# liuzuxin/FSRL

Measured on NVIDIA H100. Metric: env-steps/sec (collect+update) SafetyCarCircle-v0 PPO-Lag, higher is better.
Workload: dtype f32

## Files before the change

### fsrl_b200/csrc/ppo_persist.cu

```cuda
#include "ppo_persist.cuh"
#include "arena.cuh"
#include "ppo_loss.cuh"
#include "wgmma.cuh"
#include <cstdlib>
#include <cmath>
#include <vector>

namespace fsrl {
namespace pp {

using namespace wg;

constexpr int WQ = 2;
constexpr int NEPI = 128 * WQ;
constexpr int TPB = NEPI + 32;
constexpr int C1 = 16 / WQ;
constexpr int C2 = 32 / WQ;
constexpr int RB = 64;
constexpr int MB = 256;
constexpr int KC = 32, NCH = 256 / KC;
constexpr int SLOT_BYTES = 32768, NSLOT = 4;
constexpr int A_CHUNK = 64 * KC * 4;
constexpr int ACC_LD = 68;
constexpr int OUTP = 8;
constexpr int H_ = 256;
constexpr int IMG = 65536;
enum { I_H1A_HI, I_H1A_LO, I_H1T_HI, I_H1T_LO, I_DZA_HI, I_DZA_LO, I_DZT_HI, I_DZT_LO, I_W2A_HI, I_W2A_LO, I_W2B_HI, I_W2B_LO, N_IMG };
constexpr int DB2P_OFF = N_IMG * IMG;
constexpr int DW3P_OFF = DB2P_OFF + 4 * H_;
constexpr int DB3P_OFF = DW3P_OFF + 4 * H_ * OUTP;
constexpr int MAXD = 40;
constexpr int NSMAX = (MAXD + 1) * 32 + 32 + 32 * OUTP + 16;
constexpr int SLICE_OFF = DB3P_OFF + 4 * 16;
constexpr int NET_WS = SLICE_OFF + 8 * NSMAX;
constexpr int SUMSQ_FLOATS = 128;
constexpr int FLAG_LINE = 32;
constexpr int F_A = 0, F_C = 1, F_PER_NET = 2;
constexpr int TILE_PK = (64 * 64 / NEPI + 2) / 3;
constexpr int TILE_FLOATS = TILE_PK * NEPI * 4;
constexpr int SLICE_PK = (NSMAX + 2) / 3;
constexpr int XG_PER_NET = 16 * TILE_FLOATS + 8 * SLICE_PK * 4;
constexpr int MAX_MB = 16384;
constexpr long long WAIT_CYCLES = 6000000000LL;

struct Args {
    fsrl_ppo_update_t u;
    int n_mb, slot0;
    long long adam_t0;
    float* ws;
    unsigned* flags;
    int* err;
    const float* adam_tab;
    long long* dbg;
    int dbg_step;
    unsigned dp_seq;
    int dp_direct;
};
constexpr int DBG_N = 48;
#define STAMP(i) do { if (P.dbg && t == P.dbg_step) P.dbg[(size_t)blockIdx.x * DBG_N + (i)] = clock64(); } while (0)

struct AdamS { float w1, b2, w2, rbc2s, eps, neg_step; };
__device__ __forceinline__ float adam_one(float p, float g, float& m, float& v, const AdamS& a) {
    m = m + a.w1 * (g - m);
    v = v * a.b2 + (a.w2 * g) * g;
    const float sq = v > 0.f ? v * rsqrtf(v) : 0.f;
    const float denom = fmaf(sq, a.rbc2s, a.eps);
    return p + __fdividef(a.neg_step * m, denom);
}

__device__ __forceinline__ void fail(int* err, int code) {
    *reinterpret_cast<volatile int*>(err) = code;
    __threadfence_system();
    asm volatile("trap;");
}
__device__ __forceinline__ uint32_t pk_hash(float x, float y, float z) {
    const uint32_t a = __float_as_uint(x), b = __float_as_uint(y), c = __float_as_uint(z);
    return a ^ __funnelshift_l(b, b, 11) ^ __funnelshift_l(c, c, 22);
}
__device__ __forceinline__ bool pk_ok(const float4& v, uint32_t tag) { return (__float_as_uint(v.w) ^ pk_hash(v.x, v.y, v.z)) == tag; }
__device__ __forceinline__ void st_packet(float* p, float x, float y, float z, uint32_t tag) {
    asm volatile("st.relaxed.sys.global.v4.f32 [%0], {%1,%2,%3,%4};" ::"l"(p), "f"(x), "f"(y), "f"(z), "f"(__uint_as_float(tag ^ pk_hash(x, y, z))) : "memory");
}
__device__ __forceinline__ float4 ld_packet(const float* p) {
    float4 v;
    asm volatile("ld.relaxed.sys.global.v4.f32 {%0,%1,%2,%3}, [%4];" : "=f"(v.x), "=f"(v.y), "=f"(v.z), "=f"(v.w) : "l"(p) : "memory");
    return v;
}

__device__ __noinline__ float3 dp_gather(const float* src, long long stride, int me, int world, uint32_t tag,
                                        float ox, float oy, float oz, int* err, int code) {
    const long long t0w = clock64();
    float ax = 0.f, ay = 0.f, az = 0.f;
    for (int r0 = 0; r0 < world; r0 += 4) {
        float4 v[4];
        bool ok;
        do {
            ok = true;
#pragma unroll
            for (int k = 0; k < 4; ++k)
                if (r0 + k < world && r0 + k != me) v[k] = ld_packet(src + (size_t)(r0 + k) * stride);
#pragma unroll
            for (int k = 0; k < 4; ++k)
                if (r0 + k < world && r0 + k != me) ok = ok && pk_ok(v[k], tag);
            if (!ok && clock64() - t0w > 4 * WAIT_CYCLES) fail(err, code);
        } while (!ok);
#pragma unroll
        for (int k = 0; k < 4; ++k) {
            if (r0 + k >= world) continue;
            if (r0 + k == me) { ax += ox; ay += oy; az += oz; }
            else { ax += v[k].x; ay += v[k].y; az += v[k].z; }
        }
    }
    return make_float3(ax, ay, az);
}
__device__ __noinline__ void dp_push_all(const float* const* xg, size_t off, int me, int world, float x, float y, float z, uint32_t tag) {
    for (int r = 0; r < world; ++r)
        if (r != me) st_packet(const_cast<float*>(xg[r]) + off, x, y, z, tag);
}

__device__ __forceinline__ uint32_t mapa_u32(uint32_t local_saddr, uint32_t rank) {
// ... 218 lines not shown
__device__ __noinline__ float dp_tile_finish(DpCtx d, size_t off, float* accs, int trow, int cb2, int et) {
    float g[C2];
    const long long t0w = clock64();
    if (d.direct) {
        float own[C2];
        acc_ld<C2>(accs, trow, cb2, own);
#pragma unroll
        for (int jq = 0; jq < C2; ++jq) g[jq] = 0.f;
        for (int r = 0; r < d.world; ++r) {
            if (r == d.me) {
#pragma unroll
                for (int jq = 0; jq < C2; ++jq) g[jq] += own[jq];
                continue;
            }
            const float* src = d.xg[d.me] + (size_t)r * d.region + off;
            float4 v[TILE_PK];
            bool ok;
            do {
                ok = true;
#pragma unroll
                for (int q = 0; q < TILE_PK; ++q) v[q] = ld_packet(src + (size_t)q * NEPI * 4);
#pragma unroll
                for (int q = 0; q < TILE_PK; ++q) ok = ok && pk_ok(v[q], d.tag);
                if (!ok && clock64() - t0w > 4 * WAIT_CYCLES) fail(d.err, 42);
            } while (!ok);
#pragma unroll
            for (int q = 0; q < TILE_PK; ++q) {
                g[3 * q] += v[q].x;
                if (3 * q + 1 < C2) g[3 * q + 1] += v[q].y;
                if (3 * q + 2 < C2) g[3 * q + 2] += v[q].z;
            }
        }
        const float inv_world = 1.0f / (float)d.world;
        float sq = 0.f;
#pragma unroll
        for (int jq = 0; jq < C2; ++jq) { g[jq] *= inv_world; sq = fmaf(g[jq], g[jq], sq); }
        acc_st<C2>(accs, trow, cb2, g);
        return sq;
    }
    const float* res = d.xg[d.me] + (size_t)FSRL_P2P_MAX_RANKS * d.region + off;
    acc_ld<C2>(accs, trow, cb2, g);
    float4 v[TILE_PK];
    bool ok;
    do {
        ok = true;
#pragma unroll
        for (int q = 0; q < TILE_PK; ++q)
            if (dp_owner(et, q, d.world) != d.me) v[q] = ld_packet(res + (size_t)q * NEPI * 4);
#pragma unroll
        for (int q = 0; q < TILE_PK; ++q)
            if (dp_owner(et, q, d.world) != d.me) ok = ok && pk_ok(v[q], d.tag);
        if (!ok && clock64() - t0w > 4 * WAIT_CYCLES) fail(d.err, 42);
    } while (!ok);
    float sq = 0.f;
#pragma unroll
    for (int q = 0; q < TILE_PK; ++q) {
        if (dp_owner(et, q, d.world) == d.me) continue;
        g[3 * q] = v[q].x;
        if (3 * q + 1 < C2) g[3 * q + 1] = v[q].y;
        if (3 * q + 2 < C2) g[3 * q + 2] = v[q].z;
    }
#pragma unroll
    for (int jq = 0; jq < C2; ++jq) sq = fmaf(g[jq], g[jq], sq);
    acc_st<C2>(accs, trow, cb2, g);
    return sq;
}
__device__ __noinline__ void dp_slices(DpCtx d, size_t off_s, float* sp_g, int n, int et) {
    const int n3 = (n + 2) / 3;
    const float inv_world = 1.0f / (float)d.world;
    for (int i = et; i < n3; i += NEPI)
        dp_push_all(d.xg, (size_t)d.me * d.region + off_s + 4 * (size_t)i, d.me, d.world,
                    sp_g[3 * i], 3 * i + 1 < n ? sp_g[3 * i + 1] : 0.f, 3 * i + 2 < n ? sp_g[3 * i + 2] : 0.f, d.tag);
    const float* loc = d.xg[d.me];
    for (int i = et; i < n3; i += NEPI) {
        const float3 s3 = dp_gather(loc + off_s + 4 * (size_t)i, d.region, d.me, d.world, d.tag, sp_g[3 * i],
                                    3 * i + 1 < n ? sp_g[3 * i + 1] : 0.f, 3 * i + 2 < n ? sp_g[3 * i + 2] : 0.f, d.err, 40);
        sp_g[3 * i] = s3.x * inv_world;
        if (3 * i + 1 < n) sp_g[3 * i + 1] = s3.y * inv_world;
        if (3 * i + 2 < n) sp_g[3 * i + 2] = s3.z * inv_world;
    }
}

__device__ __forceinline__ bool red_cta() { return ((blockIdx.x >> 3) & 3) == ((blockIdx.x & 7) >> 2); }

__device__ __noinline__ float dp_tail(DpCtx d, size_t off_t, size_t off_s, float* accs, float* sp_g, int n, int trow, int cb2,
                                      int et, bool tile, bool slice) {
    if (tile && !d.direct) dp_tile_reduce(d, off_t, accs, trow, cb2, et);
    if (slice) dp_slices(d, off_s, sp_g, n, et);
    __syncwarp();
    return tile ? dp_tile_finish(d, off_t, accs, trow, cb2, et) : 0.f;
}

template <bool DP>
__global__ void __launch_bounds__(TPB, 1) ppo_persist_kernel(const Args P) {
    extern __shared__ __align__(1024) unsigned char smem_raw[];
    __shared__ __align__(8) uint64_t bar_full[NSLOT], bar_empty[NSLOT], bar_b, bar_w1;
    __shared__ float s_red[4][320];
    __shared__ float s_misc[32];
    __shared__ AdamS s_adam;
    __shared__ const float* s_xg[2][FSRL_P2P_MAX_RANKS];
    const fsrl_ppo_update_t& u = P.u;
    const int tid = threadIdx.x, warp = tid >> 5, lane = tid & 31;
    const int net = blockIdx.x >> 5, c = blockIdx.x & 31, a = c >> 3, b = c & 7;
    const bool is_g2 = c < 16;
    const int ka = (c & 15) >> 2, q4 = c & 3;

    const int D = u.D, A = u.A, C = u.C, H = H_;
    const int out = (net == 0) ? A : 1;
    const int n_cta = 32 * u.n_nets;
    float* wsn = P.ws + (size_t)net * NET_WS;
    float* sumsq_g = P.ws + (size_t)u.n_nets * NET_WS;
    unsigned* fl_net = P.flags + (size_t)net * F_PER_NET * FLAG_LINE;
    unsigned* fl_d2 = P.flags + (size_t)u.n_nets * F_PER_NET * FLAG_LINE;
    unsigned char* ring = smem_raw;
    float* accs = reinterpret_cast<float*>(smem_raw + NSLOT * SLOT_BYTES);
    float* small = accs + 64 * ACC_LD;
    const SliceMap sm(D);
    float* sp_p = small;
    float* sp_m = small + sm.n;
    float* sp_v = small + 2 * sm.n;
    float* sp_g = small + 3 * sm.n;
    float* land = small + 4 * sm.n;

    if (tid == 0) {
        for (int i = 0; i < NSLOT; ++i) { mbar_init(&bar_full[i], 1); mbar_init(&bar_empty[i], 4 * 8); }
        mbar_init(&bar_b, 1);
        mbar_init(&bar_w1, 4);
        fence_mbar_init();
    }
    __syncthreads();
    if (DP && threadIdx.x < 2 * FSRL_P2P_MAX_RANKS) s_xg[threadIdx.x / FSRL_P2P_MAX_RANKS][threadIdx.x % FSRL_P2P_MAX_RANKS] = P.u.p2p_xg[threadIdx.x / FSRL_P2P_MAX_RANKS][threadIdx.x % FSRL_P2P_MAX_RANKS];
    if (DP) __syncthreads();
    cluster_sync_all();

    const long long pbase = u.net_off[net];
    const ArenaLayout L = arena_layout(D, H, out, 0);
    const long long o_w1 = pbase + L.w1, o_b1 = pbase + L.b1, o_w2 = pbase + L.w2, o_b2 = pbase + L.b2,
                    o_w3 = pbase + L.w3, o_b3 = pbase + L.b3, o_ls = pbase + L.extra;

    if (warp == NEPI / 32) {
        if (elect_one()) {
            unsigned qq = 0;
            for (int t = 0; t < P.n_mb; ++t) {
                if (!flag_wait_ge<true>(fl_net + F_A * FLAG_LINE, 32u * (t + 1), WAIT_CYCLES)) fail(P.err, 10);
                STAMP(12);
                fence_proxy_async();
#pragma unroll 1
                for (int j = 0; j < NCH; ++j, ++qq) {
                    const int s = qq % NSLOT;
                    if (!mbar_wait(&bar_empty[s], ((qq / NSLOT) & 1) ^ 1, WAIT_CYCLES)) fail(P.err, 11);
                    unsigned char* dst = ring + (size_t)s * SLOT_BYTES;
                    mbar_expect_tx(&bar_full[s], 3 * A_CHUNK);
                    const size_t ao = (size_t)a * 16384 + (size_t)j * 64 * KC, bo = (size_t)b * 8192 + (size_t)j * 32 * KC;
                    copy_operand(dst, wsn + (size_t)I_H1A_HI * IMG + ao, A_CHUNK, &bar_full[s], 8, b, 0xff);
                    copy_operand(dst + 2 * A_CHUNK, wsn + (size_t)I_W2A_HI * IMG + bo, A_CHUNK / 2, &bar_full[s], 1, 0, 0);
                }
                STAMP(13);
                if (!flag_wait_ge<true>(fl_net + F_C * FLAG_LINE, 32u * (t + 1), WAIT_CYCLES)) fail(P.err, 12);
                STAMP(14);
                fence_proxy_async();
                const int ia = is_g2 ? I_W2B_HI : I_DZT_HI, ib = is_g2 ? I_DZA_HI : I_H1T_HI;
                const int blk_a = is_g2 ? ka : q4, blk_b = is_g2 ? q4 : ka;
                const uint16_t m4 = (uint16_t)(0xfu << (b & 4)), m2 = (uint16_t)(0x11u << (b & 3));
#pragma unroll 1
                for (int j = 0; j < NCH; ++j, ++qq) {
                    const int s = qq % NSLOT;
                    if (!mbar_wait(&bar_empty[s], ((qq / NSLOT) & 1) ^ 1, WAIT_CYCLES)) fail(P.err, 13);
                    unsigned char* dst = ring + (size_t)s * SLOT_BYTES;
                    mbar_expect_tx(&bar_full[s], 4 * A_CHUNK);
                    const size_t ao = (size_t)blk_a * 16384 + (size_t)j * 64 * KC, bo = (size_t)blk_b * 16384 + (size_t)j * 64 * KC;
                    copy_operand(dst, wsn + (size_t)ia * IMG + ao, A_CHUNK, &bar_full[s], is_g2 ? 4 : 2, is_g2 ? b & 3 : b >> 2, is_g2 ? m4 : m2);
                    copy_operand(dst + 2 * A_CHUNK, wsn + (size_t)ib * IMG + bo, A_CHUNK, &bar_full[s], is_g2 ? 2 : 4, is_g2 ? b >> 2 : b & 3, is_g2 ? m2 : m4);
                }
            }
        }
    } else {
        const int et = tid;
        const int sp = warp & 3;
        const int wq = warp >> 2;
        const int r16 = lane & 15, half = lane >> 4;
        const int trow = 16 * sp + r16;
        const int cb1 = 16 * half + C1 * wq;
        const int cb2 = 32 * half + C2 * wq;
        unsigned qq = 0;
        const uint32_t empty_r = mapa_u32(smem_u32(bar_empty), lane < 8 ? lane : 0);
        float w2p[C2], w2m[C2], w2v[C2];
        const int world = DP ? u.world : 1;
        auto dp_ctx = [&](int t_) {
            DpCtx d;
            const unsigned long long id = (unsigned long long)(P.adam_t0 + t_ + 1);
            d.xg = s_xg[(int)(id & 1ULL)];
            d.region = (long long)u.n_nets * XG_PER_NET;
            d.me = u.p2p_rank; d.world = world;
            d.tag = (P.dp_seq << 16) | (uint32_t)((t_ + 1) & 0xffff);
            d.err = P.err;
            d.direct = P.dp_direct;
            return d;
        };

        for (int i = et; i < sm.n; i += NEPI) {
            long long src = -1;
            if (i < sm.b2) { const int d = i / 32, kk = i % 32; src = (d < D) ? o_w1 + (long long)d * H + 32 * b + kk : o_b1 + 32 * b + kk; }
            else if (i < sm.w3) src = o_b2 + 32 * b + (i - sm.b2);
            else if (i < sm.b3) { const int oo = (i - sm.w3) / OUTP, jj = (i - sm.w3) % OUTP; if (jj < out) src = o_w3 + (long long)(32 * b + oo) * out + jj; }
            else { const int jj = i - sm.b3; if (jj < out) src = o_b3 + jj; else if (net == 0 && jj >= 8 && jj < 8 + A) src = o_ls + (jj - 8); }
            sp_p[i] = src >= 0 ? u.theta[src] : 0.f;
            sp_m[i] = src >= 0 ? u.adam_m[src] : 0.f;
            sp_v[i] = src >= 0 ? u.adam_v[src] : 0.f;
            sp_g[i] = 0.f;
        }
        if (!is_g2) {
            const int o = 64 * q4 + trow;
#pragma unroll
            for (int j = 0; j < C2; ++j) {
                const long long idx = o_w2 + (long long)(64 * ka + cb2 + j) * H + o;
                w2p[j] = u.theta[idx]; w2m[j] = u.adam_m[idx]; w2v[j] = u.adam_v[idx];
            }
        } else {
#pragma unroll
            for (int j = 0; j < C2; ++j) w2p[j] = w2m[j] = w2v[j] = 0.f;
        }
        epi_bar();

        for (int t = 0; t < P.n_mb; ++t) {
            const long long row0 = (long long)t * MB;
            const int slot = P.slot0 + t;
            if (et == 0) {
                s_adam.w1 = (float)(1.0 - u.beta1); s_adam.b2 = (float)u.beta2; s_adam.w2 = (float)(1.0 - u.beta2);
                s_adam.rbc2s = __ldg(P.adam_tab + 2 * t); s_adam.eps = (float)u.adam_eps; s_adam.neg_step = __ldg(P.adam_tab + 2 * t + 1);
                STAMP(0);
                if (P.dbg && t == P.dbg_step) { long long gt; asm volatile("mov.u64 %0, %%globaltimer;" : "=l"(gt)); P.dbg[(size_t)blockIdx.x * DBG_N + 30] = gt; }
                if (P.dbg && t == P.dbg_step + 64) {
                    long long gt; asm volatile("mov.u64 %0, %%globaltimer;" : "=l"(gt));
                    P.dbg[(size_t)blockIdx.x * DBG_N + 31] = gt;
                    P.dbg[(size_t)blockIdx.x * DBG_N + 29] = clock64();
                }
            }
            if (t + 1 < P.n_mb && et < 64) {
                const long long r = row0 + MB + 64 * a + et;
                prefetch_l2(u.obs + r * D);
                if (D > 32) prefetch_l2(u.obs + r * D + 32);
                if (is_g2) { prefetch_l2(u.obs + (r + 128) * D); if (D > 32) prefetch_l2(u.obs + (r + 128) * D + 32); }
                if (net == 0) { prefetch_l2(u.act + r * A); prefetch_l2(u.logp_old + r); prefetch_l2(u.adv + r); if (C > 1) prefetch_l2(u.adv + u.ld + r); }
                else { prefetch_l2(u.ret + (long long)(net - 1) * u.ld + r); if (u.value_clip) prefetch_l2(u.values + (long long)(net - 1) * u.ld + r); }
            }
            float* scratch = reinterpret_cast<float*>(ring);
            if (!is_g2) {
                const float (&pv)[C2] = w2p;
                float phi[C2], plo[C2];
                const int o = 64 * q4 + trow;
                float* w2a_hi = wsn + (size_t)I_W2A_HI * IMG + (size_t)(o >> 5) * 8192 + (size_t)(o & 31) * 4;
                float* w2a_lo = w2a_hi + IMG;
#pragma unroll
                for (int q = 0; q < C2 / 4; ++q) {
                    float4 hi, lo;
                    tf32_split(pv[4 * q], hi.x, lo.x); tf32_split(pv[4 * q + 1], hi.y, lo.y);
                    tf32_split(pv[4 * q + 2], hi.z, lo.z); tf32_split(pv[4 * q + 3], hi.w, lo.w);
                    const size_t plane = (size_t)(16 * ka + (cb2 >> 2) + q) * 128;
                    *reinterpret_cast<float4*>(w2a_hi + plane) = hi;
                    *reinterpret_cast<float4*>(w2a_lo + plane) = lo;
                    phi[4 * q] = hi.x; phi[4 * q + 1] = hi.y; phi[4 * q + 2] = hi.z; phi[4 * q + 3] = hi.w;
                    plo[4 * q] = lo.x; plo[4 * q + 1] = lo.y; plo[4 * q + 2] = lo.z; plo[4 * q + 3] = lo.w;
                }
                store_transposed<C2, 64>(scratch, phi, plo, trow, cb2, et, wsn + (size_t)I_W2B_HI * IMG + (size_t)ka * 16384, 64 * q4, 0);
            }
            if (is_g2) {
                const int r = et & 63, kc = C1 * (et >> 6);
                const float* x0 = u.obs + (row0 + 64 * a + r) * D;
                const float* x1 = u.obs + (row0 + 64 * (a + 2) + r) * D;
                float acc2[2][C1];
#pragma unroll
                for (int j = 0; j < C1; ++j) acc2[0][j] = acc2[1][j] = sp_p[sm.w1 + D * 32 + kc + j];
                for (int d = 0; d < D; ++d) {
                    const float xv0 = __ldg(x0 + d), xv1 = __ldg(x1 + d);
                    const float* w = sp_p + sm.w1 + d * 32 + kc;
#pragma unroll
                    for (int j = 0; j < C1; ++j) { acc2[0][j] = fmaf(xv0, w[j], acc2[0][j]); acc2[1][j] = fmaf(xv1, w[j], acc2[1][j]); }
                }
                constexpr int TSCR = 2 * 32 * 65;
#pragma unroll
                for (int rep = 0; rep < 2; ++rep) {
                    const int aa = a + 2 * rep;
                    float hi[C1], lo[C1];
                    float* a_hi = wsn + (size_t)I_H1A_HI * IMG + (size_t)aa * 16384 + (size_t)r * 4;
#pragma unroll
                    for (int q = 0; q < C1 / 4; ++q) {
#pragma unroll
                        for (int e = 0; e < 4; ++e) tf32_split(fmaxf(acc2[rep][4 * q + e], 0.f), hi[4 * q + e], lo[4 * q + e]);
                        const size_t plane = (size_t)(8 * b + (kc >> 2) + q) * 256;
                        *reinterpret_cast<float4*>(a_hi + plane) = make_float4(hi[4 * q], hi[4 * q + 1], hi[4 * q + 2], hi[4 * q + 3]);
                        *reinterpret_cast<float4*>(a_hi + IMG + plane) = make_float4(lo[4 * q], lo[4 * q + 1], lo[4 * q + 2], lo[4 * q + 3]);
                    }
                    transposed_stage<C1, 32>(scratch + rep * TSCR, hi, lo, r, kc);
                }
                epi_bar();
#pragma unroll
                for (int rep = 0; rep < 2; ++rep)
                    transposed_flush<32>(scratch + rep * TSCR, et, wsn + (size_t)I_H1T_HI * IMG + (size_t)(b >> 1) * 16384, 64 * (a + 2 * rep), 32 * (b & 1));
            }
            fence_proxy_async_smem();
            epi_bar();
            if (et == 0) { STAMP(1); flag_add_release(fl_net + F_A * FLAG_LINE); }

            const long long grow = row0 + 64 * a + trow;
            float p_act[8], p_lpo = 0.f, p_adv0 = 0.f, p_adv1 = 0.f, p_ret = 0.f, p_val = 0.f, mean[2] = {0.f, 0.f}, rstd[2] = {1.f, 1.f};
#pragma unroll
            for (int j = 0; j < 8; ++j) p_act[j] = 0.f;
            if (net == 0) {
#pragma unroll
                for (int j = 0; j < 8; ++j) if (j < A) p_act[j] = __ldg(u.act + grow * A + j);
                p_lpo = __ldg(u.logp_old + grow);
                p_adv0 = __ldg(u.adv + grow);
                if (C > 1) p_adv1 = __ldg(u.adv + u.ld + grow);
                const float* ms = u.mb_stats + (size_t)t * 4;
                mean[0] = __ldg(ms); rstd[0] = __ldg(ms + 1); mean[1] = __ldg(ms + 2); rstd[1] = __ldg(ms + 3);
            } else {
                p_ret = __ldg(u.ret + (long long)(net - 1) * u.ld + grow);
                if (u.value_clip) p_val = __ldg(u.values + (long long)(net - 1) * u.ld + grow);
            }
            float p_ls[8], p_rsg[8];
#pragma unroll
            for (int j = 0; j < 8; ++j) {
                p_ls[j] = (net == 0 && j < A) ? sp_p[sm.b3 + 8 + j] : 0.f;
                p_rsg[j] = 1.0f / expf(p_ls[j]);
            }

            {
                float dm[16], dc[16];
                if (wq == 0) gemm_phase<32>(ring, qq, bar_full, empty_r, dm, dc, P.err, 30, lane);
                else qq += NCH;
                stage_acc<32>(accs, dm, dc, wq, sp, lane);
            }
            if (et == 0) STAMP(2);
            float h2[C1];
            acc_ld<C1>(accs, trow, cb1, h2);
            float hp[OUTP];
#pragma unroll
            for (int j = 0; j < OUTP; ++j) hp[j] = 0.f;
#pragma unroll
            for (int j = 0; j < C1; ++j) {
                h2[j] = fmaxf(h2[j] + sp_p[sm.b2 + cb1 + j], 0.f);
                const float* w = sp_p + sm.w3 + (cb1 + j) * OUTP;
#pragma unroll
                for (int jj = 0; jj < OUTP; ++jj) hp[jj] = fmaf(h2[j], w[jj], hp[jj]);
            }
#pragma unroll
            for (int jj = 0; jj < OUTP; ++jj) hp[jj] += __shfl_xor_sync(0xffffffffu, hp[jj], 16);
            if (WQ > 1) {
                float* xh = &s_red[0][0];
                if (half == 0 && wq > 0) {
#pragma unroll
                    for (int jj = 0; jj < OUTP; ++jj) xh[((wq - 1) * 64 + trow) * OUTP + jj] = hp[jj];
                }
                epi_bar();
                if (half == 0 && wq == 0) {
#pragma unroll
                    for (int w2 = 1; w2 < WQ; ++w2)
#pragma unroll
                        for (int jj = 0; jj < OUTP; ++jj) hp[jj] += xh[((w2 - 1) * 64 + trow) * OUTP + jj];
                }
            }
            float outv[OUTP];
#pragma unroll
            for (int jj = 0; jj < OUTP; ++jj) outv[jj] = sp_p[sm.b3 + jj];
            if (et == 0) {
                STAMP(3);
                mbar_expect_tx(&bar_b, 8u * 64u * OUTP * (uint32_t)sizeof(float));
            }
            if (half == 0 && wq == 0) {
                const uint32_t mine = smem_u32(land + ((size_t)b * 64 + trow) * OUTP);
                const uint32_t bb_ = smem_u32(&bar_b);
#pragma unroll
                for (int r = 0; r < 8; ++r) {
                    const uint32_t ra = mapa_u32(mine, r), rb = mapa_u32(bb_, r);
                    st_async4(ra, make_float4(hp[0], hp[1], hp[2], hp[3]), rb);
                    st_async4(ra + 16, make_float4(hp[4], hp[5], hp[6], hp[7]), rb);
                }
            }
            if (!mbar_wait_cluster(&bar_b, t & 1, WAIT_CYCLES)) fail(P.err, 31);
            __syncwarp();
            if (et == 0) STAMP(4);
#pragma unroll
            for (int bb = 0; bb < 8; ++bb) {
                const float* src = land + ((size_t)bb * 64 + trow) * OUTP;
                const float4 v0 = *reinterpret_cast<const float4*>(src);
                const float4 v1 = *reinterpret_cast<const float4*>(src + 4);
                outv[0] += v0.x; outv[1] += v0.y; outv[2] += v0.z; outv[3] += v0.w;
                outv[4] += v1.x; outv[5] += v1.y; outv[6] += v1.z; outv[7] += v1.w;
            }
            float dd[16];
#pragma unroll
            for (int j = 0; j < 16; ++j) dd[j] = 0.f;
            float st_a = 0.f, st_b = 0.f, st_c = 0.f, st_d = 0.f;
            {
                const float invB = 1.0f / (float)MB;
                if (net == 0) {
                    float g_mu[8], g_ls[8];
                    ppo_actor_row(u, outv, p_act, p_ls, p_rsg, p_lpo, p_adv0, p_adv1, mean, rstd, invB, g_mu, g_ls,
                                  st_a, st_b, st_c);
#pragma unroll
                    for (int j = 0; j < 8; ++j) { dd[j] = g_mu[j]; dd[8 + j] = g_ls[j]; }
                } else {
                    dd[0] = ppo_value_row(u, outv[0], p_ret, p_val, invB, st_d);
                }
            }
            if (et == 0) STAMP(26);
            const int nfeed = (net == 0) ? A : 1;
            float dz[C1];
#pragma unroll
            for (int j = 0; j < C1; ++j) {
                const float* w = sp_p + sm.w3 + (cb1 + j) * OUTP;
                float g = 0.f;
#pragma unroll
                for (int jj = 0; jj < OUTP; ++jj) if (jj < nfeed) g = fmaf(dd[jj], w[jj], g);
                dz[j] = h2[j] > 0.f ? g : 0.f;
            }
            {
                float hi[C1], lo[C1];
                float* a_hi = wsn + (size_t)I_DZA_HI * IMG + (size_t)a * 16384 + (size_t)trow * 4;
#pragma unroll
                for (int q = 0; q < C1 / 4; ++q) {
#pragma unroll
                    for (int e = 0; e < 4; ++e) tf32_split(dz[4 * q + e], hi[4 * q + e], lo[4 * q + e]);
                    const size_t plane = (size_t)(8 * b + (cb1 >> 2) + q) * 256;
                    *reinterpret_cast<float4*>(a_hi + plane) = make_float4(hi[4 * q], hi[4 * q + 1], hi[4 * q + 2], hi[4 * q + 3]);
                    *reinterpret_cast<float4*>(a_hi + IMG + plane) = make_float4(lo[4 * q], lo[4 * q + 1], lo[4 * q + 2], lo[4 * q + 3]);
                }
                store_transposed<C1, 32>(scratch, hi, lo, trow, cb1, et, wsn + (size_t)I_DZT_HI * IMG + (size_t)(b >> 1) * 16384, 64 * a, 32 * (b & 1));
            }
            if (et == 0) STAMP(27);
            {
                float* row = &s_red[sp][0];
#pragma unroll
                for (int j = 0; j < C1; ++j) {
                    const float sdz = half_sum(dz[j]);
                    if (r16 == 0) row[cb1 + j] = sdz;
                }
#pragma unroll
                for (int jj = 0; jj < OUTP; ++jj) {
                    if (jj < nfeed) {
#pragma unroll
                        for (int j = 0; j < C1; ++j) {
                            const float sv = half_sum(h2[j] * dd[jj]);
                            if (r16 == 0) row[32 + 32 * jj + cb1 + j] = sv;
                        }
                    }
                }
                if (b == 0 && wq == 0) {
#pragma unroll
                    for (int j = 0; j < 16; ++j) {
                        const float sv = half_sum(dd[j]);
                        if (lane == 0) row[288 + j] = sv;
                    }
                    const float sa = half_sum(st_a), sb = half_sum(st_b), sc = half_sum(st_c), sdv = half_sum(st_d);
                    if (lane == 0) { row[304] = sa; row[305] = sb; row[306] = sc; row[307] = sdv; }
                }
            }
            epi_bar();
            if (et == 0) STAMP(28);
            for (int i = et; i < 32 + 32 * nfeed; i += NEPI) {
                const float tot = ((s_red[0][i] + s_red[1][i]) + s_red[2][i]) + s_red[3][i];
                if (i < 32) wsn[DB2P_OFF + a * H + 32 * b + i] = tot;
                else wsn[DW3P_OFF + ((size_t)a * H + 32 * b + ((i - 32) & 31)) * OUTP + ((i - 32) >> 5)] = tot;
            }
            if (b == 0) {
                if (et < 20) {
                    const int i = 288 + et;
                    const float tot = ((s_red[0][i] + s_red[1][i]) + s_red[2][i]) + s_red[3][i];
                    if (et < 16) wsn[DB3P_OFF + a * 16 + et] = tot;
                    else {
                        float* stat = u.stats + (size_t)slot * FSRL_PPO_STATS;
                        if (net == 0) { if (et == 16) atomicAdd(stat + ST_ACTOR_REW, tot); if (et == 17) atomicAdd(stat + ST_ACTOR_SAFETY, tot); if (et == 18) atomicAdd(stat + ST_KL, tot); }
                        else if (et == 19) atomicAdd(stat + ST_VF0 + (net - 1), tot);
                    }
                }
                if (net == 0 && a == 0 && et == 20) u.stats[(size_t)slot * FSRL_PPO_STATS + ST_ENTROPY] = ppo_entropy(sp_p + sm.b3 + 8, A);
            }
            fence_proxy_async_smem();
            epi_bar();
            if (et == 0) { STAMP(5); flag_add_release(fl_net + F_C * FLAG_LINE); }

            unsigned mbits = 0;
            if (is_g2) {
                const int k = 64 * ka + trow;
                const float* msk = wsn + (size_t)I_H1A_HI * IMG + (size_t)q4 * 16384 + (size_t)(k >> 2) * 256 + (k & 3);
                float mreg[C2];
#pragma unroll
                for (int jq = 0; jq < C2; ++jq) mreg[jq] = __ldcg(msk + (size_t)(cb2 + jq) * 4);
                float xr[(64 * MAXD + NEPI - 1) / NEPI];
                const int nx = (64 * D + NEPI - 1) / NEPI;
                const float* xb = u.obs + (row0 + 64 * q4) * D;
#pragma unroll
                for (int q = 0; q < (64 * MAXD + NEPI - 1) / NEPI; ++q)
                    xr[q] = (q < nx && et + q * NEPI < 64 * D) ? __ldg(xb + et + q * NEPI) : 0.f;
#pragma unroll
                for (int jq = 0; jq < C2; ++jq) mbits |= (mreg[jq] > 0.f ? 1u : 0u) << jq;
#pragma unroll
                for (int q = 0; q < (64 * MAXD + NEPI - 1) / NEPI; ++q) {
                    const int e = et + q * NEPI;
                    if (q < nx && e < 64 * D) { const int r = e / D; land[e + (r >> 5)] = xr[q]; }
                }
            }
            if (red_cta() && wq == 1) {
                const int tw = et - 128;
                if (tw == 0) {
                    if (!flag_wait_ge(fl_net + F_C * FLAG_LINE, 32u * (t + 1), WAIT_CYCLES)) fail(P.err, 35);
                    STAMP(15);
                }
                asm volatile("bar.sync 6, 128;" ::: "memory");
                for (int i0 = sm.b2 + tw; i0 < sm.n; i0 += 4 * 128) {
                    float pv[4][4];
#pragma unroll
                    for (int e = 0; e < 4; ++e) {
                        const int i = i0 + e * 128;
                        const float* src = wsn;
                        size_t stride = 0;
                        bool real = false;
                        if (i < sm.n) {
                            if (i < sm.w3) { src = wsn + DB2P_OFF + 32 * b + (i - sm.b2); stride = H; real = true; }
                            else if (i < sm.b3) {
                                const int oo = (i - sm.w3) / OUTP, jj = (i - sm.w3) % OUTP;
                                real = jj < out;
                                src = wsn + DW3P_OFF + ((size_t)32 * b + oo) * OUTP + jj; stride = (size_t)H * OUTP;
                            } else {
                                const int jj = i - sm.b3;
                                real = (jj < out) || (net == 0 && jj >= 8 && jj < 8 + A);
                                src = wsn + DB3P_OFF + jj; stride = 16;
                            }
                        }
#pragma unroll
                        for (int q = 0; q < 4; ++q) pv[e][q] = real ? __ldcg(src + q * stride) : 0.f;
                    }
#pragma unroll
                    for (int e = 0; e < 4; ++e) {
                        const int i = i0 + e * 128;
                        if (i < sm.n) {
                            float gsum = 0.f;
#pragma unroll
                            for (int q = 0; q < 4; ++q) gsum += pv[e][q];
                            sp_g[i] = gsum;
                        }
                    }
                }
                if (tw == 0) STAMP(16);
            }
            {
                float dm[32], dc[32];
                if (wq == 0) gemm_phase<64>(ring, qq, bar_full, empty_r, dm, dc, P.err, 32, lane);
                else qq += NCH;
                stage_acc<64>(accs, dm, dc, wq, sp, lane);
            }
            if (et == 0) STAMP(6);
            float sq = 0.f;
            if (is_g2) {
                float v[C2];
                acc_ld<C2>(accs, trow, cb2, v);
#pragma unroll
                for (int jq = 0; jq < C2; ++jq) v[jq] = ((mbits >> jq) & 1u) ? v[jq] : 0.f;
                epi_bar();
                if (et == 0) STAMP(22);
                const float* xh = land + (size_t)cb2 * D + half;
                float* dst = reinterpret_cast<float*>(ring) + (size_t)wq * (D + 1) * 64 + trow;
                for (int d = 0; d < D; ++d) {
                    float sacc = 0.f;
#pragma unroll
                    for (int jq = 0; jq < C2; ++jq) sacc = fmaf(xh[jq * D + d], v[jq], sacc);
                    sacc += __shfl_xor_sync(0xffffffffu, sacc, 16);
                    if (half == 0) dst[d * 64] = sacc;
                }
                float sb1 = 0.f;
#pragma unroll
                for (int jq = 0; jq < C2; ++jq) sb1 += v[jq];
                sb1 += __shfl_xor_sync(0xffffffffu, sb1, 16);
                if (half == 0) dst[D * 64] = sb1;
                if (et == 0) STAMP(23);
                epi_bar();
                if (et == 0) {
                    mbar_arrive_release_cluster(mapa_u32(smem_u32(&bar_w1), 2 * ka));
                    mbar_arrive_release_cluster(mapa_u32(smem_u32(&bar_w1), 2 * ka + 1));
                }
            } else {
                float g[C2];
                acc_ld<C2>(accs, trow, cb2, g);
                if (DP) {
                    dp_tile_send(dp_ctx(t), (size_t)(net * 16 + (c - 16)) * TILE_FLOATS + (size_t)et * 4, accs, trow, cb2, et);
                    if (et == 0) STAMP(32);
                } else {
#pragma unroll
                    for (int jq = 0; jq < C2; ++jq) sq = fmaf(g[jq], g[jq], sq);
                }
            }
            if (et == 0) STAMP(7);
            if (red_cta()) {
                if (!mbar_wait_cluster(&bar_w1, t & 1, WAIT_CYCLES)) fail(P.err, 33);
                if (et == 0) STAMP(8);
                const uint32_t ring_s = smem_u32(ring);
                const int kb = 32 * (b & 1);
                for (int i0 = et; i0 < sm.b2; i0 += 2 * NEPI) {
                    float pv[2][4 * WQ];
#pragma unroll
                    for (int e = 0; e < 2; ++e) {
                        const int i = i0 + e * NEPI;
                        const uint32_t off = 4u * (uint32_t)((i / 32) * 64 + kb + (i % 32));
#pragma unroll
                        for (int rb = 0; rb < 4; ++rb) {
                            const uint32_t src = mapa_u32(ring_s + off, (uint32_t)((4 * (b >> 1) + rb) & 7));
#pragma unroll
                            for (int w = 0; w < WQ; ++w)
                                pv[e][WQ * rb + w] = i < sm.b2 ? ld_cluster(src + 4u * (uint32_t)(w * (D + 1) * 64)) : 0.f;
                        }
                    }
#pragma unroll
                    for (int e = 0; e < 2; ++e) {
                        const int i = i0 + e * NEPI;
                        if (i < sm.b2) {
                            float gsum = 0.f;
#pragma unroll
                            for (int q = 0; q < 4 * WQ; ++q) gsum += pv[e][q];
                            sp_g[i] = gsum;
                        }
                    }
                }
                epi_bar();
                if (et == 0) STAMP(17);
            }
            if (DP) {
                const DpCtx d = dp_ctx(t);
                const size_t off_t = (size_t)(net * 16 + (c - 16)) * TILE_FLOATS + (size_t)et * 4;
                sq += dp_tail(d, off_t, (size_t)u.n_nets * 16 * TILE_FLOATS + (size_t)(net * 8 + b) * SLICE_PK * 4, accs, sp_g, sm.n,
                              trow, cb2, et, !is_g2, red_cta());
                if (et == 0) STAMP(41);
                epi_bar();
            }
            if (red_cta()) {
                for (int i = et; i < sm.n; i += NEPI) {
                    bool real = true;
                    if (i >= sm.w3 && i < sm.b3) real = ((i - sm.w3) % OUTP) < out;
                    else if (i >= sm.b3) { const int jj = i - sm.b3; real = (jj < out) || (net == 0 && jj >= 8 && jj < 8 + A); }
                    if (real && (i < sm.b3 || b == 0)) sq = fmaf(sp_g[i], sp_g[i], sq);
                    wsn[SLICE_OFF + (size_t)b * NSMAX + i] = sp_g[i];
                }
            }
            if (red_cta() || !is_g2) {
                sq = warp_sum(sq);
                if (lane == 0) s_misc[warp] = sq;
                epi_bar();
                if (et == 0) {
                    float tot = 0.f;
#pragma unroll
                    for (int w2 = 0; w2 < NEPI / 32; ++w2) tot += s_misc[w2];
                    sumsq_g[blockIdx.x - (red_cta() ? 8 * a : 0)] = tot;
                    STAMP(9);
                    flag_add_release(fl_d2);
                }
            }
            if (et == 0) {
                if (!flag_wait_ge(fl_d2, 24u * (unsigned)u.n_nets * (t + 1), WAIT_CYCLES)) fail(P.err, 34);
                STAMP(10);
            }
            epi_bar();
            float nq[4];
#pragma unroll
            for (int q = 0; q < 4; ++q) nq[q] = (lane + 32 * q < n_cta) ? __ldcg(sumsq_g + lane + 32 * q) : 0.f;
            if (!DP && !red_cta())
                for (int i = et; i < sm.n; i += NEPI) sp_g[i] = __ldcg(wsn + SLICE_OFF + (size_t)b * NSMAX + i);
            float nsq = ((nq[0] + nq[1]) + nq[2]) + nq[3];
            nsq = warp_sum(nsq);
            float gscale = 1.0f;
            if (u.max_grad_norm > 0.f) gscale = fminf(u.max_grad_norm / (sqrtf(nsq) + 1e-6f), 1.0f);
            if (blockIdx.x == 0 && et == 0) u.stats[(size_t)slot * FSRL_PPO_STATS + ST_GRADNORM] = sqrtf(nsq);
            const AdamS ad = s_adam;
            if (et == 0) STAMP(24);
            for (int i = et; i < sm.n; i += NEPI) {
                float m = sp_m[i], v = sp_v[i];
                const float g = (DP && !red_cta()) ? __ldcg(wsn + SLICE_OFF + (size_t)b * NSMAX + i) : sp_g[i];
                sp_p[i] = adam_one(sp_p[i], g * gscale, m, v, ad);
                sp_m[i] = m; sp_v[i] = v;
            }
            if (et == 0) STAMP(25);
            if (!is_g2) {
                float g[C2];
                acc_ld<C2>(accs, trow, cb2, g);
#pragma unroll
                for (int j = 0; j < C2; ++j) w2p[j] = adam_one(w2p[j], g[j] * gscale, w2m[j], w2v[j], ad);
            }
            epi_bar();
            if (et == 0) STAMP(11);
        }

        if (a == 0) {
            for (int i = et; i < sm.n; i += NEPI) {
                long long dst = -1;
                if (i < sm.b2) { const int d = i / 32, kk = i % 32; dst = (d < D) ? o_w1 + (long long)d * H + 32 * b + kk : o_b1 + 32 * b + kk; }
                else if (i < sm.w3) dst = o_b2 + 32 * b + (i - sm.b2);
                else if (i < sm.b3) { const int oo = (i - sm.w3) / OUTP, jj = (i - sm.w3) % OUTP; if (jj < out) dst = o_w3 + (long long)(32 * b + oo) * out + jj; }
                else if (b == 0) { const int jj = i - sm.b3; if (jj < out) dst = o_b3 + jj; else if (net == 0 && jj >= 8 && jj < 8 + A) dst = o_ls + (jj - 8); }
                if (dst >= 0) { u.theta[dst] = sp_p[i]; u.adam_m[dst] = sp_m[i]; u.adam_v[dst] = sp_v[i]; }
            }
        }
        if (!is_g2) {
            const int o = 64 * q4 + trow;
#pragma unroll
            for (int j = 0; j < C2; ++j) {
                const long long idx = o_w2 + (long long)(64 * ka + cb2 + j) * H + o;
                u.theta[idx] = w2p[j]; u.adam_m[idx] = w2m[j]; u.adam_v[idx] = w2v[j];
            }
        }
    }
    __syncthreads();
    cluster_sync_all();
}

static size_t smem_bytes(int D) {
    return (size_t)NSLOT * SLOT_BYTES + sizeof(float) * 64 * ACC_LD + 4 * sizeof(float) * SliceMap(D).n +
           sizeof(float) * 8 * 64 * OUTP;
}

static cudaLaunchConfig_t cluster_launch(int n_nets, size_t smem, cudaStream_t s, cudaLaunchAttribute* at) {
    at->id = cudaLaunchAttributeClusterDimension;
    at->val.clusterDim.x = 8; at->val.clusterDim.y = 1; at->val.clusterDim.z = 1;
    cudaLaunchConfig_t cfg = {};
    cfg.gridDim = dim3(32 * n_nets); cfg.blockDim = dim3(TPB); cfg.dynamicSmemBytes = smem; cfg.stream = s;
    cfg.attrs = at; cfg.numAttrs = 1;
    return cfg;
}

struct Instance {
    void (*kern)(const Args);
    int max_clusters;
};
static const Instance& instance(bool dp) {
    static Instance inst[2] = {};
    Instance& in = inst[dp];
    if (!in.kern) {
        in.kern = dp ? ppo_persist_kernel<true> : ppo_persist_kernel<false>;
        cudaLaunchAttribute at;
        const cudaLaunchConfig_t cfg = cluster_launch(1, smem_bytes(MAXD), nullptr, &at);
        if (cudaFuncSetAttribute(in.kern, cudaFuncAttributeMaxDynamicSharedMemorySize, (int)cfg.dynamicSmemBytes) != cudaSuccess ||
            cudaOccupancyMaxActiveClusters(&in.max_clusters, in.kern, &cfg) != cudaSuccess) {
            cudaGetLastError();
            in.max_clusters = 0;
        }
    }
    return in;
}

}

size_t ppo_persist_ws_floats(int n_nets, int D, int H) {
    (void)D; (void)H;
    return (size_t)n_nets * pp::NET_WS + pp::SUMSQ_FLOATS + (size_t)(n_nets * pp::F_PER_NET + 1) * pp::FLAG_LINE + 32 +
           2 * (size_t)pp::MAX_MB + 2 * (size_t)32 * n_nets * pp::DBG_N;
}

size_t ppo_persist_p2p_floats(int n_nets) { return (size_t)(FSRL_P2P_MAX_RANKS + 1) * n_nets * pp::XG_PER_NET + 64; }

bool ppo_persist_supported(const fsrl_ppo_update_t& u, long long n_total, int batch_size) {
    if (u.H != 256 || batch_size != pp::MB || n_total % pp::MB != 0 || n_total < pp::MB || n_total / pp::MB > pp::MAX_MB) return false;
    if (u.world > 1 && !(u.p2p_on && u.world <= FSRL_P2P_MAX_RANKS && (size_t)u.p2p_stride >= ppo_persist_p2p_floats(u.n_nets))) return false;
    if (u.D < 1 || u.D > pp::MAXD || u.A > 8 || u.n_nets < 1 || u.n_nets > 3) return false;
    if (u.persist_ws == nullptr || (size_t)u.persist_ws_floats < ppo_persist_ws_floats(u.n_nets, u.D, u.H)) return false;
    if (32 * u.n_nets > sm_count()) return false;
    return pp::instance(u.world > 1).max_clusters >= 4 * u.n_nets;
}

int ppo_persist_run(const fsrl_ppo_update_t& ug, int n_mb, int stats_slot0, long long adam_t0, cudaStream_t s) {
    pp::Args a;
    a.u = ug;
    a.n_mb = n_mb; a.slot0 = stats_slot0; a.adam_t0 = adam_t0;
    a.ws = ug.persist_ws;
    const size_t fl_off = (size_t)ug.n_nets * pp::NET_WS + pp::SUMSQ_FLOATS;
    a.flags = reinterpret_cast<unsigned*>(ug.persist_ws + fl_off);
    const size_t n_flag_words = (size_t)(ug.n_nets * pp::F_PER_NET + 1) * pp::FLAG_LINE;
    a.err = reinterpret_cast<int*>(a.flags + n_flag_words);
    FSRL_CUDA(cudaMemsetAsync(ug.persist_ws + fl_off - pp::SUMSQ_FLOATS, 0, (pp::SUMSQ_FLOATS + n_flag_words + 32) * sizeof(float), s));
    float* tab_dev = reinterpret_cast<float*>(a.err + 32);
    static std::vector<float> tab;
    tab.resize(2 * (size_t)n_mb);
    for (int t = 0; t < n_mb; ++t) {
        const double tt = (double)(adam_t0 + t + 1);
        const double bc1 = 1.0 - pow(ug.beta1, tt), bc2 = 1.0 - pow(ug.beta2, tt);
        tab[2 * t] = (float)(1.0 / sqrt(bc2));
        tab[2 * t + 1] = (float)(-(ug.lr / bc1));
    }
    FSRL_CUDA(cudaMemcpyAsync(tab_dev, tab.data(), tab.size() * sizeof(float), cudaMemcpyHostToDevice, s));
    a.adam_tab = tab_dev;
    static unsigned dp_seq = 0;
// ... 18 lines not shown
```

Before: 2.770 million.

## Precompute ReLU mask bitwords, prefetch obs asynchronously, and vectorize dW1 reduction

Result: faster. 2.901 million, median of 6 (+4.7%).

```diff
diff --git a/fsrl_b200/csrc/ppo_persist.cu b/fsrl_b200/csrc/ppo_persist.cu
--- a/fsrl_b200/csrc/ppo_persist.cu
+++ b/fsrl_b200/csrc/ppo_persist.cu
@@ -2,6 +2,7 @@
 #include "arena.cuh"
 #include "ppo_loss.cuh"
 #include "wgmma.cuh"
+#include <cuda_pipeline_primitives.h>
 #include <cstdlib>
 #include <cmath>
 #include <vector>
@@ -23,6 +24,7 @@
 constexpr int A_CHUNK = 64 * KC * 4;
 constexpr int ACC_LD = 68;
 constexpr int OUTP = 8;
+constexpr int XGRP = 4 * 65;
 constexpr int H_ = 256;
 constexpr int IMG = 65536;
 enum { I_H1A_HI, I_H1A_LO, I_H1T_HI, I_H1T_LO, I_DZA_HI, I_DZA_LO, I_DZT_HI, I_DZT_LO, I_W2A_HI, I_W2A_LO, I_W2B_HI, I_W2B_LO, N_IMG };
@@ -32,10 +34,11 @@
 constexpr int MAXD = 40;
 constexpr int NSMAX = (MAXD + 1) * 32 + 32 + 32 * OUTP + 16;
 constexpr int SLICE_OFF = DB3P_OFF + 4 * 16;
-constexpr int NET_WS = SLICE_OFF + 8 * NSMAX;
+constexpr int MSK_OFF = SLICE_OFF + 8 * NSMAX;
+constexpr int NET_WS = MSK_OFF + 256 * 8;
 constexpr int SUMSQ_FLOATS = 128;
 constexpr int FLAG_LINE = 32;
-constexpr int F_A = 0, F_C = 1, F_PER_NET = 2;
+constexpr int F_A = 0, F_C = 1, F_P = 2, F_PER_NET = 3;
 constexpr int TILE_PK = (64 * 64 / NEPI + 2) / 3;
 constexpr int TILE_FLOATS = TILE_PK * NEPI * 4;
 constexpr int SLICE_PK = (NSMAX + 2) / 3;
@@ -420,6 +423,9 @@
 }
 
 __device__ __forceinline__ bool red_cta() { return ((blockIdx.x >> 3) & 3) == ((blockIdx.x & 7) >> 2); }
+__device__ __forceinline__ int cb1() { return 16 * ((threadIdx.x >> 4) & 1) + C1 * (threadIdx.x >> 7); }
+__device__ __forceinline__ int cb2() { return 32 * ((threadIdx.x >> 4) & 1) + C2 * (threadIdx.x >> 7); }
+__device__ __forceinline__ int trow() { return 16 * ((threadIdx.x >> 5) & 3) + (threadIdx.x & 15); }
 
 __device__ __noinline__ float dp_tail(DpCtx d, size_t off_t, size_t off_s, float* accs, float* sp_g, int n, int trow, int cb2,
                                       int et, bool tile, bool slice) {
@@ -517,9 +523,6 @@
         const int sp = warp & 3;
         const int wq = warp >> 2;
         const int r16 = lane & 15, half = lane >> 4;
-        const int trow = 16 * sp + r16;
-        const int cb1 = 16 * half + C1 * wq;
-        const int cb2 = 32 * half + C2 * wq;
         unsigned qq = 0;
         const uint32_t empty_r = mapa_u32(smem_u32(bar_empty), lane < 8 ? lane : 0);
         float w2p[C2], w2m[C2], w2v[C2];
@@ -548,10 +551,10 @@
             sp_g[i] = 0.f;
         }
         if (!is_g2) {
-            const int o = 64 * q4 + trow;
+            const int o = 64 * q4 + trow();
 #pragma unroll
             for (int j = 0; j < C2; ++j) {
-                const long long idx = o_w2 + (long long)(64 * ka + cb2 + j) * H + o;
+                const long long idx = o_w2 + (long long)(64 * ka + cb2() + j) * H + o;
                 w2p[j] = u.theta[idx]; w2m[j] = u.adam_m[idx]; w2v[j] = u.adam_v[idx];
             }
         } else {
@@ -586,7 +589,7 @@
             if (!is_g2) {
                 const float (&pv)[C2] = w2p;
                 float phi[C2], plo[C2];
-                const int o = 64 * q4 + trow;
+                const int o = 64 * q4 + trow();
                 float* w2a_hi = wsn + (size_t)I_W2A_HI * IMG + (size_t)(o >> 5) * 8192 + (size_t)(o & 31) * 4;
                 float* w2a_lo = w2a_hi + IMG;
 #pragma unroll
@@ -594,13 +597,13 @@
                     float4 hi, lo;
                     tf32_split(pv[4 * q], hi.x, lo.x); tf32_split(pv[4 * q + 1], hi.y, lo.y);
                     tf32_split(pv[4 * q + 2], hi.z, lo.z); tf32_split(pv[4 * q + 3], hi.w, lo.w);
-                    const size_t plane = (size_t)(16 * ka + (cb2 >> 2) + q) * 128;
+                    const size_t plane = (size_t)(16 * ka + (cb2() >> 2) + q) * 128;
                     *reinterpret_cast<float4*>(w2a_hi + plane) = hi;
                     *reinterpret_cast<float4*>(w2a_lo + plane) = lo;
                     phi[4 * q] = hi.x; phi[4 * q + 1] = hi.y; phi[4 * q + 2] = hi.z; phi[4 * q + 3] = hi.w;
                     plo[4 * q] = lo.x; plo[4 * q + 1] = lo.y; plo[4 * q + 2] = lo.z; plo[4 * q + 3] = lo.w;
                 }
-                store_transposed<C2, 64>(scratch, phi, plo, trow, cb2, et, wsn + (size_t)I_W2B_HI * IMG + (size_t)ka * 16384, 64 * q4, 0);
+                store_transposed<C2, 64>(scratch, phi, plo, trow(), cb2(), et, wsn + (size_t)I_W2B_HI * IMG + (size_t)ka * 16384, 64 * q4, 0);
             }
             if (is_g2) {
                 const int r = et & 63, kc = C1 * (et >> 6);
@@ -630,6 +633,14 @@
                         *reinterpret_cast<float4*>(a_hi + IMG + plane) = make_float4(lo[4 * q], lo[4 * q + 1], lo[4 * q + 2], lo[4 * q + 3]);
                     }
                     transposed_stage<C1, 32>(scratch + rep * TSCR, hi, lo, r, kc);
+                    unsigned mw = 0;
+#pragma unroll
+                    for (int j = 0; j < C1; ++j) {
+                        const unsigned bal = __ballot_sync(0xffffffffu, hi[j] > 0.f);
+                        if (lane == j) mw = bal;
+                    }
+                    if (lane < C1)
+                        reinterpret_cast<unsigned*>(wsn + MSK_OFF)[(32 * b + kc + lane) * 8 + 2 * aa + (warp & 1)] = mw;
                 }
                 epi_bar();
 #pragma unroll
@@ -640,7 +651,7 @@
             epi_bar();
             if (et == 0) { STAMP(1); flag_add_release(fl_net + F_A * FLAG_LINE); }
 
-            const long long grow = row0 + 64 * a + trow;
+            const long long grow = row0 + 64 * a + trow();
             float p_act[8], p_lpo = 0.f, p_adv0 = 0.f, p_adv1 = 0.f, p_ret = 0.f, p_val = 0.f, mean[2] = {0.f, 0.f}, rstd[2] = {1.f, 1.f};
 #pragma unroll
             for (int j = 0; j < 8; ++j) p_act[j] = 0.f;
@@ -671,14 +682,14 @@
             }
             if (et == 0) STAMP(2);
             float h2[C1];
-            acc_ld<C1>(accs, trow, cb1, h2);
+            acc_ld<C1>(accs, trow(), cb1(), h2);
             float hp[OUTP];
 #pragma unroll
             for (int j = 0; j < OUTP; ++j) hp[j] = 0.f;
 #pragma unroll
             for (int j = 0; j < C1; ++j) {
-                h2[j] = fmaxf(h2[j] + sp_p[sm.b2 + cb1 + j], 0.f);
-                const float* w = sp_p + sm.w3 + (cb1 + j) * OUTP;
+                h2[j] = fmaxf(h2[j] + sp_p[sm.b2 + cb1() + j], 0.f);
+                const float* w = sp_p + sm.w3 + (cb1() + j) * OUTP;
 #pragma unroll
                 for (int jj = 0; jj < OUTP; ++jj) hp[jj] = fmaf(h2[j], w[jj], hp[jj]);
             }
@@ -688,14 +699,14 @@
                 float* xh = &s_red[0][0];
                 if (half == 0 && wq > 0) {
 #pragma unroll
-                    for (int jj = 0; jj < OUTP; ++jj) xh[((wq - 1) * 64 + trow) * OUTP + jj] = hp[jj];
+                    for (int jj = 0; jj < OUTP; ++jj) xh[((wq - 1) * 64 + trow()) * OUTP + jj] = hp[jj];
                 }
                 epi_bar();
                 if (half == 0 && wq == 0) {
 #pragma unroll
                     for (int w2 = 1; w2 < WQ; ++w2)
 #pragma unroll
-                        for (int jj = 0; jj < OUTP; ++jj) hp[jj] += xh[((w2 - 1) * 64 + trow) * OUTP + jj];
+                        for (int jj = 0; jj < OUTP; ++jj) hp[jj] += xh[((w2 - 1) * 64 + trow()) * OUTP + jj];
                 }
             }
             float outv[OUTP];
@@ -706,7 +717,7 @@
                 mbar_expect_tx(&bar_b, 8u * 64u * OUTP * (uint32_t)sizeof(float));
             }
             if (half == 0 && wq == 0) {
-                const uint32_t mine = smem_u32(land + ((size_t)b * 64 + trow) * OUTP);
+                const uint32_t mine = smem_u32(land + ((size_t)b * 64 + trow()) * OUTP);
                 const uint32_t bb_ = smem_u32(&bar_b);
 #pragma unroll
                 for (int r = 0; r < 8; ++r) {
@@ -720,7 +731,7 @@
             if (et == 0) STAMP(4);
 #pragma unroll
             for (int bb = 0; bb < 8; ++bb) {
-                const float* src = land + ((size_t)bb * 64 + trow) * OUTP;
+                const float* src = land + ((size_t)bb * 64 + trow()) * OUTP;
                 const float4 v0 = *reinterpret_cast<const float4*>(src);
                 const float4 v1 = *reinterpret_cast<const float4*>(src + 4);
                 outv[0] += v0.x; outv[1] += v0.y; outv[2] += v0.z; outv[3] += v0.w;
@@ -747,7 +758,7 @@
             float dz[C1];
 #pragma unroll
             for (int j = 0; j < C1; ++j) {
-                const float* w = sp_p + sm.w3 + (cb1 + j) * OUTP;
+                const float* w = sp_p + sm.w3 + (cb1() + j) * OUTP;
                 float g = 0.f;
 #pragma unroll
                 for (int jj = 0; jj < OUTP; ++jj) if (jj < nfeed) g = fmaf(dd[jj], w[jj], g);
@@ -755,24 +766,39 @@
             }
             {
                 float hi[C1], lo[C1];
-                float* a_hi = wsn + (size_t)I_DZA_HI * IMG + (size_t)a * 16384 + (size_t)trow * 4;
+                float* a_hi = wsn + (size_t)I_DZA_HI * IMG + (size_t)a * 16384 + (size_t)trow() * 4;
 #pragma unroll
                 for (int q = 0; q < C1 / 4; ++q) {
 #pragma unroll
                     for (int e = 0; e < 4; ++e) tf32_split(dz[4 * q + e], hi[4 * q + e], lo[4 * q + e]);
-                    const size_t plane = (size_t)(8 * b + (cb1 >> 2) + q) * 256;
+                    const size_t plane = (size_t)(8 * b + (cb1() >> 2) + q) * 256;
                     *reinterpret_cast<float4*>(a_hi + plane) = make_float4(hi[4 * q], hi[4 * q + 1], hi[4 * q + 2], hi[4 * q + 3]);
                     *reinterpret_cast<float4*>(a_hi + IMG + plane) = make_float4(lo[4 * q], lo[4 * q + 1], lo[4 * q + 2], lo[4 * q + 3]);
                 }
-                store_transposed<C1, 32>(scratch, hi, lo, trow, cb1, et, wsn + (size_t)I_DZT_HI * IMG + (size_t)(b >> 1) * 16384, 64 * a, 32 * (b & 1));
+                transposed_stage<C1, 32>(scratch, hi, lo, trow(), cb1());
+                epi_bar();
+                transposed_flush<32>(scratch, et, wsn + (size_t)I_DZT_HI * IMG + (size_t)(b >> 1) * 16384, 64 * a, 32 * (b & 1));
             }
             if (et == 0) STAMP(27);
+            fence_proxy_async_smem();
+            epi_bar();
+            if (et == 0) { STAMP(5); flag_add_release(fl_net + F_C * FLAG_LINE); }
+            unsigned mword = 0;
+            if (is_g2) {
+                mword = __ldcg(reinterpret_cast<const unsigned*>(wsn + MSK_OFF) + (64 * ka + trow()) * 8 + 2 * q4 + half);
+                const float* xb = u.obs + (row0 + 64 * q4) * D;
+                for (int e = et; e < 64 * D; e += NEPI) {
+                    const int r = e / D, d = e - r * D;
+                    __pipeline_memcpy_async(land + (d >> 2) * XGRP + 4 * (r + (r >> 5)) + (d & 3), xb + e, 4);
+                }
+                __pipeline_commit();
+            }
             {
                 float* row = &s_red[sp][0];
 #pragma unroll
                 for (int j = 0; j < C1; ++j) {
                     const float sdz = half_sum(dz[j]);
-                    if (r16 == 0) row[cb1 + j] = sdz;
+                    if (r16 == 0) row[cb1() + j] = sdz;
                 }
 #pragma unroll
                 for (int jj = 0; jj < OUTP; ++jj) {
@@ -780,7 +806,7 @@
 #pragma unroll
                         for (int j = 0; j < C1; ++j) {
                             const float sv = half_sum(h2[j] * dd[jj]);
-                            if (r16 == 0) row[32 + 32 * jj + cb1 + j] = sv;
+                            if (r16 == 0) row[32 + 32 * jj + cb1() + j] = sv;
                         }
                     }
                 }
@@ -814,35 +840,14 @@
                 }
                 if (net == 0 && a == 0 && et == 20) u.stats[(size_t)slot * FSRL_PPO_STATS + ST_ENTROPY] = ppo_entropy(sp_p + sm.b3 + 8, A);
             }
-            fence_proxy_async_smem();
             epi_bar();
-            if (et == 0) { STAMP(5); flag_add_release(fl_net + F_C * FLAG_LINE); }
-
-            unsigned mbits = 0;
-            if (is_g2) {
-                const int k = 64 * ka + trow;
-                const float* msk = wsn + (size_t)I_H1A_HI * IMG + (size_t)q4 * 16384 + (size_t)(k >> 2) * 256 + (k & 3);
-                float mreg[C2];
-#pragma unroll
-                for (int jq = 0; jq < C2; ++jq) mreg[jq] = __ldcg(msk + (size_t)(cb2 + jq) * 4);
-                float xr[(64 * MAXD + NEPI - 1) / NEPI];
-                const int nx = (64 * D + NEPI - 1) / NEPI;
-                const float* xb = u.obs + (row0 + 64 * q4) * D;
-#pragma unroll
-                for (int q = 0; q < (64 * MAXD + NEPI - 1) / NEPI; ++q)
-                    xr[q] = (q < nx && et + q * NEPI < 64 * D) ? __ldg(xb + et + q * NEPI) : 0.f;
-#pragma unroll
-                for (int jq = 0; jq < C2; ++jq) mbits |= (mreg[jq] > 0.f ? 1u : 0u) << jq;
-#pragma unroll
-                for (int q = 0; q < (64 * MAXD + NEPI - 1) / NEPI; ++q) {
-                    const int e = et + q * NEPI;
-                    if (q < nx && e < 64 * D) { const int r = e / D; land[e + (r >> 5)] = xr[q]; }
-                }
-            }
+            if (et == 128) { STAMP(18); flag_add_release(fl_net + F_P * FLAG_LINE); }
+
+            const unsigned mbits = (mword >> (C2 * wq)) & ((1u << C2) - 1u);
             if (red_cta() && wq == 1) {
                 const int tw = et - 128;
                 if (tw == 0) {
-                    if (!flag_wait_ge(fl_net + F_C * FLAG_LINE, 32u * (t + 1), WAIT_CYCLES)) fail(P.err, 35);
+                    if (!flag_wait_ge(fl_net + F_P * FLAG_LINE, 32u * (t + 1), WAIT_CYCLES)) fail(P.err, 35);
                     STAMP(15);
                 }
                 asm volatile("bar.sync 6, 128;" ::: "memory");
@@ -892,19 +897,34 @@
             float sq = 0.f;
             if (is_g2) {
                 float v[C2];
-                acc_ld<C2>(accs, trow, cb2, v);
+                acc_ld<C2>(accs, trow(), cb2(), v);
 #pragma unroll
                 for (int jq = 0; jq < C2; ++jq) v[jq] = ((mbits >> jq) & 1u) ? v[jq] : 0.f;
+                __pipeline_wait_prior(0);
+                if (et == 0) STAMP(19);
                 epi_bar();
                 if (et == 0) STAMP(22);
-                const float* xh = land + (size_t)cb2 * D + half;
-                float* dst = reinterpret_cast<float*>(ring) + (size_t)wq * (D + 1) * 64 + trow;
-                for (int d = 0; d < D; ++d) {
-                    float sacc = 0.f;
-#pragma unroll
-                    for (int jq = 0; jq < C2; ++jq) sacc = fmaf(xh[jq * D + d], v[jq], sacc);
-                    sacc += __shfl_xor_sync(0xffffffffu, sacc, 16);
-                    if (half == 0) dst[d * 64] = sacc;
+                const float* xh = land + 4 * (cb2() + half);
+                float* dst = reinterpret_cast<float*>(ring) + (size_t)wq * (D + 1) * 64 + trow();
+                for (int d = 0; d < D; d += 4, xh += XGRP) {
+                    float sacc[4] = {0.f, 0.f, 0.f, 0.f};
+#pragma unroll 1
+                    for (int h = 0; h < 2; ++h) {
+                        float vh[C2 / 2];
+#pragma unroll
+                        for (int jq = 0; jq < C2 / 2; ++jq) vh[jq] = h ? v[C2 / 2 + jq] : v[jq];
+#pragma unroll
+                        for (int jq = 0; jq < C2 / 2; ++jq) {
+                            const float4 x = *reinterpret_cast<const float4*>(xh + 4 * (C2 / 2 * h + jq));
+                            sacc[0] = fmaf(x.x, vh[jq], sacc[0]); sacc[1] = fmaf(x.y, vh[jq], sacc[1]);
+                            sacc[2] = fmaf(x.z, vh[jq], sacc[2]); sacc[3] = fmaf(x.w, vh[jq], sacc[3]);
+                        }
+                    }
+#pragma unroll
+                    for (int e = 0; e < 4; ++e) {
+                        sacc[e] += __shfl_xor_sync(0xffffffffu, sacc[e], 16);
+                        if (half == 0 && d + e < D) dst[(d + e) * 64] = sacc[e];
+                    }
                 }
                 float sb1 = 0.f;
 #pragma unroll
@@ -919,9 +939,9 @@
                 }
             } else {
                 float g[C2];
-                acc_ld<C2>(accs, trow, cb2, g);
+                acc_ld<C2>(accs, trow(), cb2(), g);
                 if (DP) {
-                    dp_tile_send(dp_ctx(t), (size_t)(net * 16 + (c - 16)) * TILE_FLOATS + (size_t)et * 4, accs, trow, cb2, et);
+                    dp_tile_send(dp_ctx(t), (size_t)(net * 16 + (c - 16)) * TILE_FLOATS + (size_t)et * 4, accs, trow(), cb2(), et);
                     if (et == 0) STAMP(32);
                 } else {
 #pragma unroll
@@ -966,7 +986,7 @@
                 const DpCtx d = dp_ctx(t);
                 const size_t off_t = (size_t)(net * 16 + (c - 16)) * TILE_FLOATS + (size_t)et * 4;
                 sq += dp_tail(d, off_t, (size_t)u.n_nets * 16 * TILE_FLOATS + (size_t)(net * 8 + b) * SLICE_PK * 4, accs, sp_g, sm.n,
-                              trow, cb2, et, !is_g2, red_cta());
+                              trow(), cb2(), et, !is_g2, red_cta());
                 if (et == 0) STAMP(41);
                 epi_bar();
             }
@@ -1018,7 +1038,7 @@
             if (et == 0) STAMP(25);
             if (!is_g2) {
                 float g[C2];
-                acc_ld<C2>(accs, trow, cb2, g);
+                acc_ld<C2>(accs, trow(), cb2(), g);
 #pragma unroll
                 for (int j = 0; j < C2; ++j) w2p[j] = adam_one(w2p[j], g[j] * gscale, w2m[j], w2v[j], ad);
             }
@@ -1037,10 +1057,10 @@
             }
         }
         if (!is_g2) {
-            const int o = 64 * q4 + trow;
+            const int o = 64 * q4 + trow();
 #pragma unroll
             for (int j = 0; j < C2; ++j) {
-                const long long idx = o_w2 + (long long)(64 * ka + cb2 + j) * H + o;
+                const long long idx = o_w2 + (long long)(64 * ka + cb2() + j) * H + o;
                 u.theta[idx] = w2p[j]; u.adam_m[idx] = w2m[j]; u.adam_v[idx] = w2v[j];
             }
         }
```
